# loryruta/gl-radix-sort

Hardware: AMD Instinct MI355X
Metric: Mkeys/s sorting 2^28 uint32 key+val; % HBM roofline; 1/2/4/8 GPU (higher is better)
Workload: dtype u32; 1 GPU; 2^28 uint32 key + uint32 val pairs, uniform-random full-range keys, vals=iota, in-place stable radix sort, 1x MI355X; pairs_per_gpu=268435456, key_distribution=uniform, parallelism=single, device=AMD Radeon Graphics (gfx950:sramecc+:xnack-), 256 CUs, 288.0 GiB, device 0

## Files before the change

### gl-radix-sort_amd/csrc/radix_lds_bucket.hpp

```cpp
#pragma once

#include "radix_lds_finish.hpp"

namespace glu_hip
{
constexpr uint32_t bucket_ceil_log2(uint32_t v)
{
    uint32_t b = 0;
    while ((1u << b) < v) b++;
    return b;
}
constexpr uint32_t bucket_floor_pow2(uint32_t v)
{
    uint32_t p = 1;
    while (p * 2 <= v) p *= 2;
    return p;
}

constexpr uint32_t kBucketMaxLen = 24;
template<typename KeyT>
constexpr bool bucket_late_values()
{
#ifdef GLU_BUCKET_LATE_VALUES
    return GLU_BUCKET_LATE_VALUES != 0;
#else
    return sizeof(KeyT) == 4;
#endif
}

template<typename KeyT, int THREADS, int KPT, bool VALS>
struct BucketSmem
{
    using WordT = KeyT;
    static constexpr int WAVES = THREADS / kWave;
    static constexpr int TILE = THREADS * KPT;
    static constexpr int FRONT = 32;
    static constexpr int CAP = TILE + FRONT;
    static constexpr int SLOT_BITS = (int) bucket_ceil_log2(CAP);
    static constexpr int NB = (int) bucket_floor_pow2(TILE);
    static constexpr int DIGIT_BITS = (int) bucket_ceil_log2(NB);
    static constexpr int BPT = NB / THREADS;
    static constexpr int EPV = 16 / (int) sizeof(KeyT);
    static constexpr int KV = (CAP / EPV + THREADS - 1) / THREADS;
    static constexpr int VQ = (CAP / 4 + THREADS - 1) / THREADS;
    static constexpr int ITEMS = KV * EPV;
    static_assert(CAP % 4 == 0 && BPT >= 4 && BPT % 4 == 0, "bucket geometry");
    union
    {
        alignas(16) uint32_t hist[NB + 4];
        alignas(16) uint32_t vstage[VALS ? CAP : 4];
    } a;
    alignas(16) WordT wstage[CAP + 12];
    uint32_t scan_tmp[WAVES];
    uint32_t crowded;
    KeyT run_hi;
};
static_assert(sizeof(BucketSmem<uint32_t, 256, 18, true>) <= 40 * 1024, "four workgroups per CU");
static_assert(sizeof(BucketSmem<uint32_t, 512, 18, true>) <= 80 * 1024, "two workgroups per CU");
static_assert(sizeof(BucketSmem<uint64_t, 512, 9, true>) <= 80 * 1024, "64-bit keys: two workgroups per CU");

#ifndef GLU_BUCKET_WAVES_PER_SIMD
#define GLU_BUCKET_WAVES_PER_SIMD 4
#endif
template<typename KeyT, int THREADS, int KPT, bool VALS, bool LOOP, bool XF = false>
__global__ __launch_bounds__(THREADS, GLU_BUCKET_WAVES_PER_SIMD) void radix_finish_bucket_kernel(KeyT* keys_a, uint32_t* vals_a, KeyT* keys_b, uint32_t* vals_b,
                                                                      const uint32_t* __restrict__ starts, uint32_t low_bits,
                                                                      const PassPlan* plan, uint32_t pass, uint32_t geometry,
                                                                      uint32_t key_xf = 0, uint32_t nruns = kFinishRuns,
                                                                      uint32_t* __restrict__ crowded = nullptr)
{
    typedef uint32_t u32x4_t __attribute__((ext_vector_type(4)));
    using Smem = BucketSmem<KeyT, THREADS, KPT, VALS>;
    using WordT = typename Smem::WordT;
    constexpr int WAVES = Smem::WAVES;
    constexpr int CAP = Smem::CAP, SB = Smem::SLOT_BITS, NB = Smem::NB, DB = Smem::DIGIT_BITS, BPT = Smem::BPT;
    constexpr int EPV = Smem::EPV, KV = Smem::KV, VQ = Smem::VQ, ITEMS = Smem::ITEMS;
    constexpr uint32_t SMASK = (1u << SB) - 1u;
    constexpr WordT INVALID = (WordT) ~(WordT) 0;
    constexpr bool kBucketLateValues = bucket_late_values<KeyT>();
    if (plan->top_bit) low_bits = plan->top_bit - 16u;
    const KeyCodec<KeyT, XF> codec_out(key_xf);
    if (plan->finish != geometry) return;
    if (plan->finish_rounds) return;

    KeyT* const keys = plan->flip[pass] ? keys_b : keys_a;
    uint32_t* const vals = plan->flip[pass] ? vals_b : vals_a;
    extern __shared__ __attribute__((aligned(16))) unsigned char smem_raw[];
    Smem& s = *reinterpret_cast<Smem*>(smem_raw);
    const uint32_t tid = threadIdx.x, lane = tid & 63, wave = tid >> 6;
    const uint32_t n = starts[nruns];
    const KeyT low_mask = low_bits >= 8u * sizeof(KeyT) ? (KeyT) ~(KeyT) 0 : (KeyT) ((((KeyT) 1) << low_bits) - 1);
    const uint32_t dsh = low_bits + SB > (uint32_t) DB ? low_bits + SB - DB : 0u;

    for (uint32_t run = blockIdx.x; run < nruns; run += LOOP ? gridDim.x : nruns)
    {
    const uint32_t begin = starts[run], end = starts[run + 1];
    const uint32_t len = end - begin;
    if (len == 0 || (!XF && len == 1)) continue;
    if (len > (uint32_t) Smem::TILE) continue;
    const uint32_t front = begin & 31u, f4 = front & 3u;
    const uint32_t abegin = begin - front;
    const uint32_t total = front + len;

    u32x4_t kraw[KV];
#pragma unroll
    for (int r = 0; r < KV; r++)
    {
        const uint32_t q = r * THREADS + tid, e0 = abegin + q * EPV;
        kraw[r] = u32x4_t{0u, 0u, 0u, 0u};
        if (q * EPV < total && e0 + EPV <= n) kraw[r] = *reinterpret_cast<const u32x4_t*>(keys + e0);
    }
    u32x4_t vraw[VALS ? VQ : 1];
    auto load_values = [&]() {
#pragma unroll
        for (int r = 0; r < VQ; r++)
        {
            const uint32_t q = r * THREADS + tid, e0 = abegin + q * 4u;
            vraw[r] = u32x4_t{0u, 0u, 0u, 0u};
            if (q * 4u < total && e0 + 4u <= n) vraw[r] = *reinterpret_cast<const u32x4_t*>(vals + e0);
        }
        if (abegin + ((total + 3u) & ~3u) > n)
        {
#pragma unroll
            for (int r = 0; r < VQ; r++)
            {
                const uint32_t q = r * THREADS + tid, e0 = abegin + q * 4u;
                if (q * 4u < total && e0 + 4u > n)
                {
                    uint32_t t[4];
#pragma unroll
                    for (int e = 0; e < 4; e++) t[e] = e0 + e < n ? vals[e0 + e] : 0u;
                    __builtin_memcpy(&vraw[r], t, 16);
                }
            }
        }
    };
    if (VALS && !kBucketLateValues) load_values();
    if (abegin + ((total + 3u) & ~3u) > n)
    {
#pragma unroll
        for (int r = 0; r < KV; r++)
        {
            const uint32_t q = r * THREADS + tid, e0 = abegin + q * EPV;
            if (q * EPV < total && e0 + EPV > n)
            {
                KeyT t[EPV];
#pragma unroll
                for (int e = 0; e < EPV; e++) t[e] = e0 + e < n ? keys[e0 + e] : (KeyT) 0;
                __builtin_memcpy(&kraw[r], t, 16);
            }
        }
    }
    {
        const u32x4_t z = {0u, 0u, 0u, 0u};
#pragma unroll
        for (int j = 0; j < BPT / 4; j++) *reinterpret_cast<u32x4_t*>(&s.a.hist[(j * THREADS + tid) * 4]) = z;
        if (tid == 0) *reinterpret_cast<u32x4_t*>(&s.a.hist[NB]) = z, s.crowded = 0u;
    }
    const uint32_t wave_s = (uint32_t) __builtin_amdgcn_readfirstlane((int) wave);
    auto live = [&](int r) { return (r * THREADS + wave_s * kWave) * EPV < total; };
    WordT word[ITEMS];
#pragma unroll
    for (int r = 0; r < KV; r++)
    {
        KeyT t[EPV];
        __builtin_memcpy(t, &kraw[r], 16);
#pragma unroll
        for (int e = 0; e < EPV; e++)
        {
            const uint32_t slot = (r * THREADS + tid) * EPV + e;
            const bool valid = slot >= front && slot < total;
            word[r * EPV + e] = valid ? (WordT) (((WordT) (t[e] & low_mask) << SB) | (WordT) slot) : INVALID;
            if (slot == front) s.run_hi = (KeyT) (t[e] & ~low_mask);
        }
    }
    __syncthreads();
    uint32_t place[ITEMS];
    bool crowded_seen = false;
    {
        const bool v0 = word[0] != INVALID;
        const uint64_t vm = __ballot(v0);
        if (vm != 0ull)
        {
            const uint32_t d0 = (uint32_t) (word[0] >> dsh);
            const uint32_t lead = (uint32_t) __builtin_amdgcn_readlane((int) d0, (int) __builtin_ctzll(vm));
            constexpr int kSameBucket = NB >= 4096 ? 4 : NB >= 2048 ? 6 : 8;
            if (__popcll(__ballot(v0 && d0 == lead)) >= kSameBucket)
            {
                crowded_seen = true;
                if (lane == 0) s.crowded = 1u;
            }
        }
    }
#pragma unroll
    for (int r = 0; r < KV; r++)
    {
#pragma unroll
        for (int e = 0; e < EPV; e++) place[r * EPV + e] = 0u;
        if (live(r) && !crowded_seen)
        {
            if (r == 1 || r == 2) crowded_seen = __builtin_amdgcn_readfirstlane((int) *(volatile uint32_t*) &s.crowded) != 0;
            if (!crowded_seen)
            {
                uint32_t worst = 0;
#pragma unroll
                for (int e = 0; e < EPV; e++)
                {
                    const int i = r * EPV + e;
                    if (word[i] != INVALID) place[i] = atomicAdd(&s.a.hist[(uint32_t) (word[i] >> dsh)], 1u);
                    worst = max(worst, place[i]);
                }
                if (__ballot(worst >= kBucketMaxLen) != 0ull)
                {
                    crowded_seen = true;
                    if (lane == 0) s.crowded = 1u;
                }
            }
        }
    }
    __syncthreads();
    if (s.crowded != 0u)
    {
        if (tid == 0) crowded_list_append(crowded, nruns, run);
        if (LOOP) __syncthreads();
        continue;
    }
    {
        uint32_t c[BPT];
#pragma unroll
        for (int j = 0; j < BPT / 4; j++)
        {
            const u32x4_t v = *reinterpret_cast<const u32x4_t*>(&s.a.hist[tid * BPT + j * 4]);
            c[j * 4 + 0] = v.x, c[j * 4 + 1] = v.y, c[j * 4 + 2] = v.z, c[j * 4 + 3] = v.w;
        }
        uint32_t sum = 0;
#pragma unroll
        for (int j = 0; j < BPT; j++)
        {
            const uint32_t t = c[j];
            c[j] = sum | (t << 16);
            sum += t;
        }
        uint32_t wtotal;
        const uint32_t excl = wave_exclusive_sum(sum, lane, wtotal);
        if (lane == 0) s.scan_tmp[wave] = wtotal;
        __syncthreads();
        uint32_t base = f4 + excl;
#pragma unroll
        for (int w = 0; w < WAVES; w++) base += (uint32_t) w < wave ? s.scan_tmp[w] : 0u;
#pragma unroll
        for (int j = 0; j < BPT / 4; j++)
        {
            const u32x4_t v = {base + c[j * 4 + 0], base + c[j * 4 + 1], base + c[j * 4 + 2], base + c[j * 4 + 3]};
            *reinterpret_cast<u32x4_t*>(&s.a.hist[tid * BPT + j * 4]) = v;
        }
    }
    __syncthreads();
    auto values_to_slots = [&]() {
#pragma unroll
        for (int r = 0; r < VQ; r++)
        {
            const uint32_t q = r * THREADS + tid;
            if (q * 4u < total) *reinterpret_cast<u32x4_t*>(&s.a.vstage[q * 4u]) = vraw[r];
        }
    };
    {
#pragma unroll
        for (int r = 0; r < KV; r++)
        {
            if (!live(r)) continue;
#pragma unroll
            for (int e = 0; e < EPV; e++)
            {
                const int i = r * EPV + e;
                if (word[i] != INVALID) s.wstage[(s.a.hist[(uint32_t) (word[i] >> dsh)] & 0xFFFFu) + place[i]] = word[i];
            }
        }
        __syncthreads();
        if (VALS && kBucketLateValues) load_values();
        uint32_t hm_next = s.a.hist[tid];
#pragma unroll 1
        for (int j = 0; j < BPT; j++)
        {
            const uint32_t hm = hm_next;
            if (j + 1 < BPT) hm_next = s.a.hist[(j + 1) * THREADS + tid];
            const uint32_t st = hm & 0xFFFFu, m = hm >> 16;
            if (m >= 2u)
            {
                auto cx = [](WordT& a, WordT& b) {
                    const WordT lo = a < b ? a : b, hi = a < b ? b : a;
                    a = lo, b = hi;
                };
                if (m <= 4u)
                {
                    WordT x0 = s.wstage[st], x1 = s.wstage[st + 1], x2 = s.wstage[st + 2], x3 = s.wstage[st + 3];
                    x2 = m > 2u ? x2 : INVALID;
                    x3 = m > 3u ? x3 : INVALID;
                    cx(x0, x1), cx(x2, x3), cx(x0, x2), cx(x1, x3), cx(x1, x2);
                    s.wstage[st] = x0, s.wstage[st + 1] = x1;
                    if (m > 2u) s.wstage[st + 2] = x2;
                    if (m > 3u) s.wstage[st + 3] = x3;
                }
                else if (m <= 8u)
                {
                    WordT x[8];
#pragma unroll
                    for (int e = 0; e < 8; e++) x[e] = s.wstage[st + e];
#pragma unroll
                    for (int e = 5; e < 8; e++) x[e] = m > (uint32_t) e ? x[e] : INVALID;
                    cx(x[0], x[1]), cx(x[2], x[3]), cx(x[4], x[5]), cx(x[6], x[7]);
                    cx(x[0], x[2]), cx(x[1], x[3]), cx(x[4], x[6]), cx(x[5], x[7]);
                    cx(x[1], x[2]), cx(x[5], x[6]);
                    cx(x[0], x[4]), cx(x[1], x[5]), cx(x[2], x[6]), cx(x[3], x[7]);
                    cx(x[2], x[4]), cx(x[3], x[5]);
                    cx(x[1], x[2]), cx(x[3], x[4]), cx(x[5], x[6]);
#pragma unroll
                    for (int e = 0; e < 8; e++)
                        if (m > (uint32_t) e) s.wstage[st + e] = x[e];
                }
                else
                {
                    for (uint32_t a = st + 1u; a < st + m; a++)
                    {
                        const WordT x = s.wstage[a];
                        uint32_t b = a;
                        while (b > st)
                        {
                            const WordT y = s.wstage[b - 1u];
                            if (y < x) break;
                            s.wstage[b] = y;
                            b--;
                        }
                        s.wstage[b] = x;
                    }
                }
            }
        }
        if (VALS)
        {
            __syncthreads();
            values_to_slots();
        }
    }
    __syncthreads();
    {
        const KeyT run_hi = s.run_hi;
        const uint32_t pieces = (f4 + len + 3u) / 4u;
        const uint32_t ebase = begin - f4;
        for (uint32_t j = tid; j < pieces; j += THREADS)
        {
            WordT w4[4];
            if constexpr (sizeof(WordT) == 4)
            {
                const u32x4_t v = *reinterpret_cast<const u32x4_t*>(&s.wstage[j * 4]);
                w4[0] = v.x, w4[1] = v.y, w4[2] = v.z, w4[3] = v.w;
            }
            else
            {
                const u32x4_t v0 = *reinterpret_cast<const u32x4_t*>(&s.wstage[j * 4]);
                const u32x4_t v1 = *reinterpret_cast<const u32x4_t*>(&s.wstage[j * 4 + 2]);
                w4[0] = (WordT) v0.x | ((WordT) v0.y << 32), w4[1] = (WordT) v0.z | ((WordT) v0.w << 32);
                w4[2] = (WordT) v1.x | ((WordT) v1.y << 32), w4[3] = (WordT) v1.z | ((WordT) v1.w << 32);
            }
            KeyT k4[4];
            uint32_t v4[4];
#pragma unroll
            for (int e = 0; e < 4; e++)
            {
                k4[e] = codec_out.decode((KeyT) (run_hi | (KeyT) ((w4[e] >> SB) & low_mask)));
                v4[e] = VALS ? s.a.vstage[(uint32_t) w4[e] & SMASK] : 0u;
            }
            const uint32_t p0 = j * 4u;
            if (p0 >= f4 && p0 + 4u <= f4 + len)
            {
                if constexpr (sizeof(KeyT) == 4)
                {
                    const u32x4_t kv = {(uint32_t) k4[0], (uint32_t) k4[1], (uint32_t) k4[2], (uint32_t) k4[3]};
                    __builtin_nontemporal_store(kv, reinterpret_cast<u32x4_t*>(keys + ebase + p0));
                }
                else
                {
                    const u32x4_t ka = {(uint32_t) k4[0], (uint32_t) ((uint64_t) k4[0] >> 32), (uint32_t) k4[1], (uint32_t) ((uint64_t) k4[1] >> 32)};
                    const u32x4_t kb = {(uint32_t) k4[2], (uint32_t) ((uint64_t) k4[2] >> 32), (uint32_t) k4[3], (uint32_t) ((uint64_t) k4[3] >> 32)};
                    __builtin_nontemporal_store(ka, reinterpret_cast<u32x4_t*>(keys + ebase + p0));
                    __builtin_nontemporal_store(kb, reinterpret_cast<u32x4_t*>(keys + ebase + p0 + 2));
                }
                if (VALS)
                {
                    const u32x4_t vv = {v4[0], v4[1], v4[2], v4[3]};
                    __builtin_nontemporal_store(vv, reinterpret_cast<u32x4_t*>(vals + ebase + p0));
                }
            }
            else
            {
#pragma unroll
                for (int e = 0; e < 4; e++)
                {
                    const uint32_t p = p0 + e;
                    if (p >= f4 && p < f4 + len)
                    {
                        __builtin_nontemporal_store(k4[e], &keys[ebase + p]);
                        if (VALS) __builtin_nontemporal_store(v4[e], &vals[ebase + p]);
                    }
                }
            }
        }
    }
    if (LOOP) __syncthreads();
    }
}

}
```

Baseline: 74500 Mkeys/s.

## Build compact work lists of multi-element buckets for the in-LDS fixup sort

```diff
diff --git a/gl-radix-sort_amd/csrc/radix_lds_bucket.hpp b/gl-radix-sort_amd/csrc/radix_lds_bucket.hpp
--- a/gl-radix-sort_amd/csrc/radix_lds_bucket.hpp
+++ b/gl-radix-sort_amd/csrc/radix_lds_bucket.hpp
@@ -27,6 +27,21 @@
     return sizeof(KeyT) == 4;
 #endif
 }
+
+constexpr uint32_t kBucketListCap = 1408;
+constexpr uint32_t kBucketRareCap = 224;
+template<int NB, int SLOT_BITS>
+constexpr bool bucket_lists()
+{
+#ifdef GLU_BUCKET_LISTS
+    return GLU_BUCKET_LISTS != 0 && NB <= 4096 && SLOT_BITS + 2 <= 16;
+#else
+    return NB <= 4096 && SLOT_BITS + 2 <= 16;
+#endif
+}
+#if (defined(GLU_BUCKET_TUNE_NO_STEP3) || defined(GLU_BUCKET_TUNE_NO_WIDE) || defined(GLU_BUCKET_TUNE_NO_INSERT)) && !defined(GLU_BUCKET_TUNING_TOOL)
+#error "GLU_BUCKET_TUNE_NO_*: tuning builds of tools/finish_bucket_bench.hip only (wrong results)"
+#endif
 
 template<typename KeyT, int THREADS, int KPT, bool VALS>
 struct BucketSmem
@@ -44,6 +59,7 @@
     static constexpr int KV = (CAP / EPV + THREADS - 1) / THREADS;
     static constexpr int VQ = (CAP / 4 + THREADS - 1) / THREADS;
     static constexpr int ITEMS = KV * EPV;
+    static constexpr bool LISTS = bucket_lists<NB, SLOT_BITS>();
     static_assert(CAP % 4 == 0 && BPT >= 4 && BPT % 4 == 0, "bucket geometry");
     union
     {
@@ -52,7 +68,10 @@
     } a;
     alignas(16) WordT wstage[CAP + 12];
     uint32_t scan_tmp[WAVES];
+    uint32_t nrare;
     uint32_t crowded;
+    uint32_t list_rare[LISTS ? kBucketRareCap : 1];
+    uint16_t list_main[LISTS ? kBucketListCap : 2];
     KeyT run_hi;
 };
 static_assert(sizeof(BucketSmem<uint32_t, 256, 18, true>) <= 40 * 1024, "four workgroups per CU");
@@ -73,7 +92,9 @@
     using Smem = BucketSmem<KeyT, THREADS, KPT, VALS>;
     using WordT = typename Smem::WordT;
     constexpr int WAVES = Smem::WAVES;
-    constexpr int CAP = Smem::CAP, SB = Smem::SLOT_BITS, NB = Smem::NB, DB = Smem::DIGIT_BITS, BPT = Smem::BPT;
+    constexpr int SB = Smem::SLOT_BITS, NB = Smem::NB, DB = Smem::DIGIT_BITS, BPT = Smem::BPT;
+    constexpr bool LISTS = Smem::LISTS;
+    static_assert(!LISTS || (int) kBucketRareCap <= THREADS, "the rare list: one entry per thread at the most");
     constexpr int EPV = Smem::EPV, KV = Smem::KV, VQ = Smem::VQ, ITEMS = Smem::ITEMS;
     constexpr uint32_t SMASK = (1u << SB) - 1u;
     constexpr WordT INVALID = (WordT) ~(WordT) 0;
@@ -155,7 +176,7 @@
         const u32x4_t z = {0u, 0u, 0u, 0u};
 #pragma unroll
         for (int j = 0; j < BPT / 4; j++) *reinterpret_cast<u32x4_t*>(&s.a.hist[(j * THREADS + tid) * 4]) = z;
-        if (tid == 0) *reinterpret_cast<u32x4_t*>(&s.a.hist[NB]) = z, s.crowded = 0u;
+        if (tid == 0) *reinterpret_cast<u32x4_t*>(&s.a.hist[NB]) = z, s.crowded = 0u, s.nrare = 0u;
     }
     const uint32_t wave_s = (uint32_t) __builtin_amdgcn_readfirstlane((int) wave);
     auto live = [&](int r) { return (r * THREADS + wave_s * kWave) * EPV < total; };
@@ -225,6 +246,7 @@
         if (LOOP) __syncthreads();
         continue;
     }
+    uint32_t nmain = 0;
     {
         uint32_t c[BPT];
 #pragma unroll
@@ -238,16 +260,40 @@
         for (int j = 0; j < BPT; j++)
         {
             const uint32_t t = c[j];
-            c[j] = sum | (t << 16);
+            c[j] = (sum & 0xFFFFu) | (t << 16);
             sum += t;
+            if constexpr (LISTS) sum += t - 2u <= 2u ? 0x10000u : 0u;
         }
         uint32_t wtotal;
         const uint32_t excl = wave_exclusive_sum(sum, lane, wtotal);
         if (lane == 0) s.scan_tmp[wave] = wtotal;
         __syncthreads();
-        uint32_t base = f4 + excl;
-#pragma unroll
-        for (int w = 0; w < WAVES; w++) base += (uint32_t) w < wave ? s.scan_tmp[w] : 0u;
+        uint32_t before = excl, all = 0;
+#pragma unroll
+        for (int w = 0; w < WAVES; w++)
+        {
+            const uint32_t t = s.scan_tmp[w];
+            before += (uint32_t) w < wave ? t : 0u;
+            all += t;
+        }
+        const uint32_t base = f4 + (before & 0xFFFFu);
+        if constexpr (LISTS)
+        {
+            nmain = (uint32_t) __builtin_amdgcn_readfirstlane((int) (all >> 16));
+            const bool fits = nmain <= kBucketListCap;
+            uint32_t at = before >> 16;
+#pragma unroll
+            for (int j = 0; j < BPT; j++)
+            {
+                const uint32_t m = c[j] >> 16, st = base + (c[j] & 0xFFFFu);
+                if (fits && m - 2u <= 2u) s.list_main[at++] = (uint16_t) (st | ((m - 2u) << SB));
+                if (m > 4u)
+                {
+                    const uint32_t r = atomicAdd(&s.nrare, 1u);
+                    if (r < kBucketRareCap) s.list_rare[r] = st | (m << 16);
+                }
+            }
+        }
 #pragma unroll
         for (int j = 0; j < BPT / 4; j++)
         {
@@ -276,69 +322,113 @@
                 if (word[i] != INVALID) s.wstage[(s.a.hist[(uint32_t) (word[i] >> dsh)] & 0xFFFFu) + place[i]] = word[i];
             }
         }
+        if (VALS && tid < 4u)
+        {
+            if (tid < f4) s.wstage[tid] = (WordT) 0;
+            if (f4 + len + tid < ((f4 + len + 3u) & ~3u)) s.wstage[f4 + len + tid] = (WordT) 0;
+        }
         __syncthreads();
         if (VALS && kBucketLateValues) load_values();
-        uint32_t hm_next = s.a.hist[tid];
+        auto cx = [](WordT& a, WordT& b) {
+            const WordT lo = a < b ? a : b, hi = a < b ? b : a;
+            a = lo, b = hi;
+        };
+        auto order_few = [&](uint32_t st, uint32_t m) {
+            WordT x0 = s.wstage[st], x1 = s.wstage[st + 1], x2 = s.wstage[m > 2u ? st + 2u : st], x3 = s.wstage[m > 3u ? st + 3u : st];
+            x2 = m > 2u ? x2 : INVALID;
+            x3 = m > 3u ? x3 : INVALID;
+            cx(x0, x1), cx(x2, x3), cx(x0, x2), cx(x1, x3), cx(x1, x2);
+            s.wstage[st] = x0, s.wstage[st + 1] = x1;
+            if (m > 2u) s.wstage[st + 2] = x2;
+            if (m > 3u) s.wstage[st + 3] = x3;
+        };
+        auto order_many = [&](uint32_t st, uint32_t m) {
+            if (m <= 8u)
+            {
+#ifndef GLU_BUCKET_TUNE_NO_WIDE
+                WordT x[8];
+#pragma unroll
+                for (int e = 0; e < 5; e++) x[e] = s.wstage[st + e];
+#pragma unroll
+                for (int e = 5; e < 8; e++)
+                {
+                    x[e] = s.wstage[m > (uint32_t) e ? st + e : st];
+                    x[e] = m > (uint32_t) e ? x[e] : INVALID;
+                }
+                cx(x[0], x[1]), cx(x[2], x[3]), cx(x[4], x[5]), cx(x[6], x[7]);
+                cx(x[0], x[2]), cx(x[1], x[3]), cx(x[4], x[6]), cx(x[5], x[7]);
+                cx(x[1], x[2]), cx(x[5], x[6]);
+                cx(x[0], x[4]), cx(x[1], x[5]), cx(x[2], x[6]), cx(x[3], x[7]);
+                cx(x[2], x[4]), cx(x[3], x[5]);
+                cx(x[1], x[2]), cx(x[3], x[4]), cx(x[5], x[6]);
+#pragma unroll
+                for (int e = 0; e < 8; e++)
+                    if (m > (uint32_t) e) s.wstage[st + e] = x[e];
+#endif
+            }
+            else
+            {
+#ifndef GLU_BUCKET_TUNE_NO_INSERT
+                for (uint32_t a = st + 1u; a < st + m; a++)
+                {
+                    const WordT x = s.wstage[a];
+                    uint32_t b = a;
+                    while (b > st)
+                    {
+                        const WordT y = s.wstage[b - 1u];
+                        if (y < x) break;
+                        s.wstage[b] = y;
+                        b--;
+                    }
+                    s.wstage[b] = x;
+                }
+#endif
+            }
+        };
+        bool every = true;
+        uint32_t nrare = 0;
+        if constexpr (LISTS)
+        {
+            nrare = (uint32_t) __builtin_amdgcn_readfirstlane((int) s.nrare);
+            every = nmain > kBucketListCap || nrare > kBucketRareCap;
+        }
+#ifndef GLU_BUCKET_TUNE_NO_STEP3
+        if (every)
+        {
+            uint32_t hm_next = s.a.hist[tid];
 #pragma unroll 1
-        for (int j = 0; j < BPT; j++)
-        {
-            const uint32_t hm = hm_next;
-            if (j + 1 < BPT) hm_next = s.a.hist[(j + 1) * THREADS + tid];
-            const uint32_t st = hm & 0xFFFFu, m = hm >> 16;
-            if (m >= 2u)
-            {
-                auto cx = [](WordT& a, WordT& b) {
-                    const WordT lo = a < b ? a : b, hi = a < b ? b : a;
-                    a = lo, b = hi;
-                };
-                if (m <= 4u)
-                {
-                    WordT x0 = s.wstage[st], x1 = s.wstage[st + 1], x2 = s.wstage[st + 2], x3 = s.wstage[st + 3];
-                    x2 = m > 2u ? x2 : INVALID;
-                    x3 = m > 3u ? x3 : INVALID;
-                    cx(x0, x1), cx(x2, x3), cx(x0, x2), cx(x1, x3), cx(x1, x2);
-                    s.wstage[st] = x0, s.wstage[st + 1] = x1;
-                    if (m > 2u) s.wstage[st + 2] = x2;
-                    if (m > 3u) s.wstage[st + 3] = x3;
-                }
-                else if (m <= 8u)
-                {
-                    WordT x[8];
-#pragma unroll
-                    for (int e = 0; e < 8; e++) x[e] = s.wstage[st + e];
-#pragma unroll
-                    for (int e = 5; e < 8; e++) x[e] = m > (uint32_t) e ? x[e] : INVALID;
-                    cx(x[0], x[1]), cx(x[2], x[3]), cx(x[4], x[5]), cx(x[6], x[7]);
-                    cx(x[0], x[2]), cx(x[1], x[3]), cx(x[4], x[6]), cx(x[5], x[7]);
-                    cx(x[1], x[2]), cx(x[5], x[6]);
-                    cx(x[0], x[4]), cx(x[1], x[5]), cx(x[2], x[6]), cx(x[3], x[7]);
-                    cx(x[2], x[4]), cx(x[3], x[5]);
-                    cx(x[1], x[2]), cx(x[3], x[4]), cx(x[5], x[6]);
-#pragma unroll
-                    for (int e = 0; e < 8; e++)
-                        if (m > (uint32_t) e) s.wstage[st + e] = x[e];
-                }
-                else
-                {
-                    for (uint32_t a = st + 1u; a < st + m; a++)
-                    {
-                        const WordT x = s.wstage[a];
-                        uint32_t b = a;
-                        while (b > st)
-                        {
-                            const WordT y = s.wstage[b - 1u];
-                            if (y < x) break;
-                            s.wstage[b] = y;
-                            b--;
-                        }
-                        s.wstage[b] = x;
-                    }
-                }
-            }
-        }
+            for (int j = 0; j < BPT; j++)
+            {
+                const uint32_t hm = hm_next;
+                if (j + 1 < BPT) hm_next = s.a.hist[(j + 1) * THREADS + tid];
+                const uint32_t st = hm & 0xFFFFu, m = hm >> 16;
+                if (m >= 2u)
+                {
+                    if (m <= 4u)
+                        order_few(st, m);
+                    else
+                        order_many(st, m);
+                }
+            }
+        }
+        else if constexpr (LISTS)
+        {
+#pragma unroll 1
+            for (uint32_t i = tid; i < nmain; i += THREADS)
+            {
+                const uint32_t e = s.list_main[i];
+                order_few(e & SMASK, 2u + (e >> SB));
+            }
+            if (wave_s * kWave < nrare && tid < nrare)
+            {
+                const uint32_t hm = s.list_rare[tid];
+                order_many(hm & 0xFFFFu, hm >> 16);
+            }
+        }
+#endif
         if (VALS)
         {
-            __syncthreads();
+            if (every) __syncthreads();
             values_to_slots();
         }
     }
```

Result: no change. 74460 Mkeys/s (-0.1%).
